# smithlabcode/abismal

Measured on AMD Instinct MI355X. Metric: mapped reads/sec (whole node), 100 bp SE on hg38-scale index, higher is better.
Workload: dtype u64

## Files before the change

### abismal_amd/csrc/abm_kernels.hip

```cpp
#include <type_traits>
#include "abm_kernels_core.hpp"
#include "abm_sam.hpp"

#ifndef ABM_SE_WAVES_PER_SIMD
#define ABM_SE_WAVES_PER_SIMD 5
#endif


namespace abm {

__global__ __launch_bounds__(256) void pack_reads_kernel(const char *__restrict__ blob,
                                                         const u64 *__restrict__ off, u64 n_reads,
                                                         u32 W, u64 *__restrict__ packed,
                                                         u32 *__restrict__ lens) {
  const u64 gid = static_cast<u64>(blockIdx.x) * blockDim.x + threadIdx.x;
  const u64 r = gid / W;
  const u32 w = static_cast<u32>(gid % W);
  if (r >= n_reads)
    return;
  const u64 b = off[r];
  const u32 L = static_cast<u32>(off[r + 1] - b);
  if (w == 0)
    lens[r] = L;
  u64 ft = 0, fa = 0, rt = 0, ra = 0;
// ... 30 lines not shown
  if (b >= n_blocks) return;
  u64 lo = 0, hi = 0;
  bool multi = false, blank = false;
  for (u32 k = 0; k < 4; ++k) {
    const u64 w = 4 * b + k;
    const u64 x = w < n_words ? genome[w] : 0ull;
    lo |= static_cast<u64>(every_fourth_bit((x >> 1) | (x >> 3))) << (16 * k);
    hi |= static_cast<u64>(every_fourth_bit((x >> 2) | (x >> 3))) << (16 * k);
    const u64 ones = (x & 0x1111111111111111ull) + ((x >> 1) & 0x1111111111111111ull) +
                     ((x >> 2) & 0x1111111111111111ull) + ((x >> 3) & 0x1111111111111111ull);
    u64 part = 0x1111111111111111ull;
    const u64 first = 16 * w;
    if (first >= n_bases) part = 0;
    else if (n_bases - first < 16) part &= (1ull << (4 * (n_bases - first))) - 1;
    if (ones & (part * 14ull)) multi = true;
    if ((~(ones | (ones >> 1) | (ones >> 2)) & part) != 0) blank = true;
  }
  p0[2 * b] = lo; p0[2 * b + 1] = hi;
  p1[2 * b] = lo; p1[2 * b + 1] = hi;
  if (multi) atomicOr(bad, 1u);
  if (blank) {
    const u64 at = b * kPlaneBlock, from = at >= kPlaneReach ? at - kPlaneReach : 0;
    for (u64 c = from >> kPlaneChunkBits; c <= (at + kPlaneBlock - 1) >> kPlaneChunkBits; ++c)
      atomicOr(&nmap[c >> 5], 1u << (c & 31u));
  }
}

template <bool BAM>
__device__ __forceinline__ u32 format_sam_tail(const SeArgs &a, u8 *line , const u32 *fin, u64 r,
                                               u32 L, const Hit &best, u32 n_ops) {
  const bool ambig = (best.flags & kFlagAmbig) != 0;
  if (best.pos == 0 || L == 0 || (ambig && !a.sam_allow_ambig)) return 0;
  if (n_ops == 0 || n_ops > a.cig_stride || n_ops > kSeCap) return 0xFFFFFFFFu;
  wave_sync();
  const u32 reflen = sam_ref_len(fin, n_ops);
  u32 chrom = 0, c0 = 0;
  if (!sam_locate(a.ix, best.pos, reflen, chrom, c0)) return 0;
  const bool rc = (best.flags & kFlagRC) != 0;
  const u32 flag = (rc ? 0x10u : 0u) | ((a.sam_allow_ambig && ambig) ? 0x100u : 0u);
  if constexpr (BAM) {
    const BamFields f{static_cast<int>(chrom) - 1, best.pos - c0, reflen, flag, -1, 0u, 0, best.diffs, (best.flags & kFlagARich) != 0};
    return BamWriter{line, a.sam_stride}.write(f, fin, n_ops, a.blob + a.off[r], L, rc, a.sam_tail + r * a.sam_stride);
  }
  SamWriter o{line, 0, a.sam_stride};
  o.put('\t');
  o.put_uint(flag);
  o.put('\t');
  o.put_chrom(a.ix, chrom);
  o.put('\t');
  o.put_uint(best.pos - c0 + 1u);
  o.put_str("\t255\t", 5);
  o.put_cigar(fin, n_ops);
  o.put_str("\t*\t0\t0\t", 7);
  o.put_seq(a.blob + a.off[r], L, rc);
  o.put_tags(best.diffs, (best.flags & kFlagARich) != 0);
  if (o.w > o.cap) return 0xFFFFFFFFu;
  o.flush(reinterpret_cast<u32 *>(a.sam_tail + r * a.sam_stride));
  return o.w;
}

template <bool TIMED, bool COOP, bool LONG, bool REC = false, bool BAM = false>
__device__ __forceinline__ void map_se_body(const SeArgs &a) {
  extern __shared__ __align__(16) unsigned char smem[];
  const int lane = lane_id();
  WaveLds lds;
  lds.W = a.W;
  lds.WB = a.WB;
  lds.qpk = reinterpret_cast<u64 *>(smem);
  lds.GW = a.GW;
  lds.qbits = lds.qpk + 4 * a.W;
  lds.MB = LONG ? 0u : (a.max_len + kPlaneBlock - 1) / kPlaneBlock;
  lds.qmask = lds.qbits + 4 * a.WB;
  lds.max_jobs = LONG ? 2u : kMaxJobs;
  {
    unsigned char *p = reinterpret_cast<unsigned char *>(lds.qmask + 4 * lds.MB * 4);
    const u32 cap2 = (a.ctmp_cap + 1) & ~1u;
    if (LONG) lds.ctmp = a.long_ctmp + static_cast<u64>(blockIdx.x) * cap2;
    else { lds.ctmp = reinterpret_cast<u32 *>(p); p += cap2 * 4; }
    lds.jpos = reinterpret_cast<u32 *>(p); p += kSeCap * 4;
    lds.jdf = reinterpret_cast<u32 *>(p); p += kSeCap * 4;
    lds.gwin = reinterpret_cast<u64 *>(p); p += lds.max_jobs * a.GW * 8;
    lds.pcache = reinterpret_cast<u64 *>(p); p += (8u << kPosCacheBits) + (LONG ? 0u : a.tb_extra);
    lds.tb = LONG ? a.long_tb + static_cast<u64>(blockIdx.x) * a.long_tb_bytes : reinterpret_cast<u8 *>(lds.gwin + a.GW);
    lds.lbest = reinterpret_cast<int *>(p); p += 64 * 4;
    lds.smark = reinterpret_cast<u32 *>(p); p += 128 * 4;
    lds.sdelta = reinterpret_cast<u32 *>(p); p += 128 * 4;
    lds.mark = reinterpret_cast<u16 *>(p);
  }
  lds.hres = reinterpret_cast<u16 *>(lds.lbest);
  lds.G = a.G;
  lds.smark[lane] = 0; lds.smark[64 + lane] = 0;
  u32 seg_epoch = 0;

  const u32 n_calls = a.mode == 2 ? 4u : 2u;
  const u32 call_rc = a.mode == 2 ? 0xCu  : 0x2u ;
  const u32 call_ar = a.mode == 2 ? 0x6u  : (a.mode == 1 ? 0x3u : 0x0u);

  WorkTally wt = {0, 0, 0, 0, 0, 0, 0, 0, 0, 0, 0, 0, 0, 0};
  const CigarSink sink = {a.cig_stride, a.ctmp_cap, a.cig_arena, a.cig_arena_count, a.cig_arena_cap, (!LONG && a.sam_tail) ? lds.jpos : nullptr};
  const u64 n_items = a.n_reads;
  long long t_begin = 0, t_a = 0, t_b = 0;
  ABM_STAMP(t_begin);
  u32 n_aln = 0, n_single = 0;
  bool overflow = false, too_long = false;

  const u64 dealt = gridDim.x;
  auto next_read = [&]() -> u64 {
    unsigned long long v = 0;
    if (lane == 0) {
      v = atomicAdd(a.next_read, 1ull) + dealt;
      if (v >= n_items && a.drained) __hip_atomic_store(a.drained, 1u, __ATOMIC_RELAXED, __HIP_MEMORY_SCOPE_SYSTEM);
    }
    return (static_cast<u64>(static_cast<u32>(uni(static_cast<int>(v >> 32)))) << 32) |
           static_cast<u32>(uni(static_cast<int>(v)));
  };
  u64 r_next = blockIdx.x;
  while (r_next < n_items) {
    const u64 slot = r_next;
    const u64 r = a.order ? static_cast<u64>(a.order[r_next]) : r_next;
    r_next = next_read();
    __builtin_amdgcn_s_setprio(0);
    long long t_read = 0;
    if (TIMED) t_read = clock64();
    bool rd_overflow = false;
    const u32 L = a.lens[r];
    Hit best;
    best.diffs = 0x7fff; best.flags = 0; best.pos = 0;
    u32 n_ops = 0;
    u32 *cig_out = a.cig + r * a.cig_stride;
    if (L > kMaxReadLen) too_long = true;
    if (L >= a.ix.min_len && L <= a.max_len) {
      const u64 *src = a.packed + (LONG ? slot : r) * 4 * a.W;
      for (u32 k = lane; k < 4 * a.W; k += 64) lds.qpk[k] = src[k];
      wave_sync();
      for (u32 e = 0; e < 4; ++e)
        for (u32 wb = 0; wb < a.WB; ++wb) {
          const u32 j = wb * 64 + lane;
          const bool b = j < L ? bit2(q_nibble(lds.qpk + e * a.W, j)) : true;
          const u64 word = __ballot(b);
          if (lane == 0) lds.qbits[e * a.WB + wb] = word;
        }
      if constexpr (COOP) build_qmasks(lds, L);
      wave_sync();
      if (L < max(a.ix.window, L >> 1) + kKeyWeight - 1)
        ghost_bits(a.packed, a.lens, r, L, a.max_len, a.ix.min_len, a.W, a.WB, lds.qbits);

      SeSet S;
      S.begin_read(L);
      for (u32 cidx = 0; cidx < n_calls; ++cidx) {
        const bool rc = (call_rc >> cidx) & 1u, ar = (call_ar >> cidx) & 1u;
        const bool g_to_a = rc != ar;
        const u32 enc = (rc ? 2u : 0u) + (g_to_a ? 1u : 0u);
        const u32 flags = (rc ? kFlagRC : 0u) | (ar ? kFlagARich : 0u);
        S.cutoff = S.good_cutoff;
        seed_pass<true, TIMED, COOP, REC>(a.ix, lds, enc, g_to_a, flags, L, S, wt, seg_epoch);
        if (S.sz != static_cast<int>(kSeCap) || S.cutoff > S.good_cutoff) {
          S.cutoff = S.top_d();
          seed_pass<false, TIMED, COOP, REC>(a.ix, lds, enc, g_to_a, flags, L, S, wt, seg_epoch);
        }
      }
      ABM_STAMP(t_a);
      choose_se<LONG>(a.ix, lds, L, a.valid_frac, S, best, cig_out, sink, n_ops, rd_overflow, n_aln, n_single);
      overflow |= rd_overflow;
      ABM_STAMP(t_b);
      if (TIMED) wt.t_align += t_b - t_a;
    }
    if constexpr (!LONG) {
      if (a.sam_tail != nullptr) {
        const u32 len = (L > a.max_len) ? 0xFFFFFFFFu : format_sam_tail<BAM>(a, lds.tb, lds.jpos, r, (L >= a.ix.min_len) ? L : 0u, best, best.pos != 0 ? n_ops : 0u);
        if (lane == 0) store_out(a.sam_len + r, len);
      }
    }
    if (lane == 0) {
      store_out(a.res + r, best);
      store_out(a.cig_n + r, best.pos != 0 ? n_ops : 0u);
      if (TIMED && a.read_cycles) a.read_cycles[r] = static_cast<u32>((clock64() - t_read) >> 10);
    }
    if (!LONG && a.slice_left != nullptr) {
      __builtin_amdgcn_fence(__ATOMIC_RELEASE, "workgroup");
      asm volatile("s_waitcnt vmcnt(0)" ::: "memory");
      if (lane == 0 && !rd_overflow) {
        const u32 sl = a.slice_id[r];
        if (sl != 0xFFFFu && atomicSub(&a.slice_left[sl], 1u) == 1u) {
          __threadfence_system();
          __hip_atomic_store(a.slice_done + sl, 1u, __ATOMIC_RELAXED, __HIP_MEMORY_SCOPE_SYSTEM);
        }
      }
    }
  }
  if (TIMED && a.work) {
    auto wsum = [&](u32 v) { u32 t; (void)wave_excl_sum(v, t); return t; };
    const u32 s0 = wsum(wt.seed_iters), s1 = wsum(wt.probes), s2 = wsum(wt.cands), s3 = wsum(wt.words);
    const u32 wsum_hits = wsum(wt.cache_hits);
    if (lane == 0) {
      atomicAdd(&a.work[0], static_cast<unsigned long long>(s0));
      atomicAdd(&a.work[1], static_cast<unsigned long long>(s1));
      atomicAdd(&a.work[2], static_cast<unsigned long long>(s2));
      atomicAdd(&a.work[3], static_cast<unsigned long long>(s3));
      atomicAdd(&a.work[4], static_cast<unsigned long long>(wt.updates));
      atomicAdd(&a.work[5], static_cast<unsigned long long>(n_aln));
      atomicAdd(&a.work[11], static_cast<unsigned long long>(wsum_hits));
      atomicAdd(&a.work[12], static_cast<unsigned long long>(n_single));
      if (TIMED) {
        atomicAdd(&a.work[6], static_cast<unsigned long long>(wt.t_probe));
        atomicAdd(&a.work[7], static_cast<unsigned long long>(wt.t_stream));
        atomicAdd(&a.work[8], static_cast<unsigned long long>(wt.t_replay));
        atomicAdd(&a.work[9], static_cast<unsigned long long>(wt.t_align));
        atomicAdd(&a.work[10], static_cast<unsigned long long>(phase_stamp() - t_begin));
        atomicAdd(&a.work[13], static_cast<unsigned long long>(wt.light_steps));
        atomicAdd(&a.work[14], static_cast<unsigned long long>(wt.fifo_updates));
        atomicAdd(&a.work[15], static_cast<unsigned long long>(wt.steps));
      }
    }
  }
  if (lane == 0 && (overflow || too_long))
    atomicOr(a.status, (overflow ? 1u : 0u) | (too_long ? 2u : 0u));
  if (a.host_tail != nullptr && lane == 0) {
    __threadfence();
    const u32 before = atomicAdd(a.finished, 1u);
    if (before + 1u == gridDim.x) {
      __threadfence();
      a.host_tail[0] = __hip_atomic_load(a.cig_arena_count, __ATOMIC_RELAXED, __HIP_MEMORY_SCOPE_AGENT);
      a.host_tail[1] = __hip_atomic_load(a.status, __ATOMIC_RELAXED, __HIP_MEMORY_SCOPE_AGENT);
    }
  }
}

template <bool TIMED, bool COOP, bool REC = false>
__global__ __launch_bounds__(64, ABM_SE_WAVES_PER_SIMD) void map_se_kernel(SeArgs a) { map_se_body<TIMED, COOP, false, REC>(a); }
template <bool COOP, bool REC>
__global__ __launch_bounds__(64, ABM_SE_WAVES_PER_SIMD) void map_se_bam_kernel(SeArgs a) { map_se_body<false, COOP, false, REC, true>(a); }
__global__ __launch_bounds__(64, 1) void map_se_long_kernel(SeArgs a) { map_se_body<false, false, true>(a); }

__global__ __launch_bounds__(256) void collect_long_kernel(const u32 *__restrict__ lens, u64 n, u32 *__restrict__ list,
                                                           u32 *__restrict__ count) {
  const u64 r = static_cast<u64>(blockIdx.x) * blockDim.x + threadIdx.x;
  if (r < n && lens[r] > kLdsReadLen && lens[r] <= kMaxReadLen) list[atomicAdd(count, 1u)] = static_cast<u32>(r);
}
__global__ __launch_bounds__(256) void pack_listed_kernel(const char *__restrict__ blob, const u64 *__restrict__ off,
                                                          const u32 *__restrict__ list, u64 m, u32 W, u64 *__restrict__ packed) {
  const u64 gid = static_cast<u64>(blockIdx.x) * blockDim.x + threadIdx.x;
  const u64 slot = gid / W;
  const u32 w = static_cast<u32>(gid % W);
  if (slot >= m) return;
  const u64 r = list[slot];
  const u64 b = off[r];
  const u32 L = static_cast<u32>(off[r + 1] - b);
  u64 ft = 0, fa = 0, rt = 0, ra = 0;
  for (u32 j = 0; j < 16; ++j) {
    const u32 k = w * 16 + j;
    u32 nft = 15, nfa = 15, nrt = 15, nra = 15;
    if (k < L) {
      const u32 cf = static_cast<u8>(blob[b + k]);
      const u32 cr = comp_base(static_cast<u8>(blob[b + (L - 1 - k)]));
      nft = read_nibble(cf, false); nfa = read_nibble(cf, true);
      nrt = read_nibble(cr, false); nra = read_nibble(cr, true);
    }
    const u32 sh = j << 2;
    ft |= static_cast<u64>(nft) << sh; fa |= static_cast<u64>(nfa) << sh;
    rt |= static_cast<u64>(nrt) << sh; ra |= static_cast<u64>(nra) << sh;
  }
  if (w * 16 >= L) ft = fa = rt = ra = ~0ull;
  u64 *dst = packed + (slot * 4) * W + w;
  dst[0] = ft; dst[W] = fa; dst[2 * W] = rt; dst[3 * W] = ra;
}

__device__ __forceinline__ u32 weight_class(const DevIndex &ix, const u64 *pk, u32 L, bool g_to_a) {
  u32 k2 = 0, k3 = 0;
  const u64 w0 = pk[0], w1 = L > 16 ? pk[1] : 0ull;
  for (u32 j = 0; j < kKeyWeight; ++j) {
    const u32 nb = static_cast<u32>((j < 16 ? w0 >> (j << 2) : w1 >> ((j - 16) << 2))) & 15u;
    k2 = (k2 << 1) | bit2(nb);
  }
  for (u32 j = 0; j < kKeyWeight3; ++j)
    k3 = k3 * 3u + trit(static_cast<u32>(w0 >> (j << 2)) & 15u, g_to_a);
  const u32 *cnt3 = g_to_a ? ix.counter_a : ix.counter_t;
  const u32 occ = (ix.counter[k2 + 1] - ix.counter[k2]) + (cnt3[k3 + 1] - cnt3[k3]);
  return 32u - static_cast<u32>(__clz(static_cast<int>(occ | 1u)));
}

__global__ __launch_bounds__(256) void weigh_reads_kernel(DevIndex ix, const u64 *__restrict__ packed,
                                                          const u32 *__restrict__ lens, u64 n, u32 W,
                                                          int mode, u8 *__restrict__ cls,
                                                          u32 *__restrict__ class_count) {
  __shared__ u32 hist[33];
  if (threadIdx.x < 33) hist[threadIdx.x] = 0;
  __syncthreads();
  const u64 r = static_cast<u64>(blockIdx.x) * blockDim.x + threadIdx.x;
  if (r < n) {
    const u32 L = lens[r];
    u32 c = 0;
    if (L >= ix.min_len) {
      const u64 *pk = packed + r * 4 * W;
      const bool ar = mode == 1;
      c = max(weight_class(ix, pk + (ar ? 1 : 0) * W, L, ar), weight_class(ix, pk + (2 + (ar ? 0 : 1)) * W, L, !ar));
    }
    cls[r] = static_cast<u8>(c);
    atomicAdd(&hist[c], 1u);
  }
  __syncthreads();
  if (threadIdx.x < 33 && hist[threadIdx.x]) atomicAdd(&class_count[threadIdx.x], hist[threadIdx.x]);
}

__global__ void order_bases_kernel(u32 *class_count ) {
  if (threadIdx.x == 0 && blockIdx.x == 0) {
    u32 at = 0;
    for (int c = 32; c >= 0; --c) { const u32 k = class_count[c]; class_count[c] = at; at += k; }
// ... 283 lines not shown
```

### abismal_amd/csrc/abm_kernels_core.hpp

```cpp
#pragma once
#include "abm_kernels.hpp"

namespace abm {

struct SeSet {
  static constexpr bool kFifo = true;
  static constexpr bool kAppend = false;
  int hk;
  u32 pf;
  u32 pp;
  int sz, cutoff, good_cutoff;
  int best_d;
  u32 best_f, best_p;
  bool sure_ambig;

  __device__ __forceinline__ static int key_d(int k) { return k >> 8; }
  __device__ __forceinline__ void begin_read(u32 readlen) {
    const int worst = static_cast<i16>(0.4 * readlen);
    hk = worst * 256; pf = 0; pp = 0;
    sz = 1;
    cutoff = worst;
    good_cutoff = static_cast<i16>(readlen / 10u);
    best_d = worst; best_f = 0; best_p = 0;
    sure_ambig = false;
  }
  __device__ __forceinline__ int top_d() const { return key_d(rdlane(hk, 0)); }
  __device__ __forceinline__ void sift_up(int hole, int key) {
    int parent = (hole - 1) / 2;
    while (hole > 0) {
      const int pk = rdlane(hk, parent);
      if (!(key_d(pk) < key_d(key))) break;
      wrlane(hk, hole, pk);
      hole = parent;
      parent = (hole - 1) / 2;
    }
    wrlane(hk, hole, key);
  }
  __device__ __forceinline__ int pop_max(int n) {
    const int len = n - 1;
    const int freed = rdlane(hk, 0) & 255;
    const int vk = rdlane(hk, len);
    int hole = 0, second = 0;
    while (second < (len - 1) / 2) {
      second = 2 * (second + 1);
      int sk = rdlane(hk, second);
      const int lk = rdlane(hk, second - 1);
      if (key_d(sk) < key_d(lk)) { --second; sk = lk; }
      wrlane(hk, hole, sk);
      hole = second;
    }
    if ((len & 1) == 0 && second == (len - 2) / 2) {
      second = 2 * (second + 1);
      wrlane(hk, hole, rdlane(hk, second - 1));
      hole = second - 1;
    }
    sift_up(hole, vk);
    return freed;
  }
  __device__ __forceinline__ int replace_top(int d, u32 f, u32 p) {
    static_assert(kSeCap == 50, "paths derived for a 50-element heap");
    const int left = __builtin_amdgcn_update_dpp(0, hk, 0x138 , 0xf, 0xf, false);
    const u64 right_wins = __ballot(!(key_d(hk) < key_d(left)));
    auto down = [&](int node) { const int r = 2 * node + 2; return ((right_wins >> r) & 1ull) ? r : r - 1; };
    const int root = rdlane(hk, 0), vk = rdlane(hk, 49);
    const int p1 = down(0), p2 = down(p1), p3 = down(p2), p4 = down(p3);
    const bool five = p4 < 24;
    const int p5 = five ? down(p4) : 63;
    const int k1 = rdlane(hk, p1), k2 = rdlane(hk, p2), k3 = rdlane(hk, p3), k4 = rdlane(hk, p4), k5 = rdlane(hk, p5);
    const int dv = key_d(vk);
    int j = 0;
    if (key_d(k1) >= dv) j = 1;
    if (key_d(k2) >= dv) j = 2;
    if (key_d(k3) >= dv) j = 3;
    if (key_d(k4) >= dv) j = 4;
    if (five && key_d(k5) >= dv) j = 5;
    wrlane(hk, 0, j == 0 ? vk : k1);
    wrlane(hk, p1, j > 1 ? k2 : (j == 1 ? vk : k1));
    wrlane(hk, p2, j > 2 ? k3 : (j == 2 ? vk : k2));
    wrlane(hk, p3, j > 3 ? k4 : (j == 3 ? vk : k3));
    wrlane(hk, p4, j > 4 ? k5 : (j == 4 ? vk : k4));
    wrlane(hk, p5, j == 5 ? vk : k5);
    const int slot = root & 255;
    wrlane(pf, slot, f);
    wrlane(pp, slot, p);
    const int nk = d * 256 + slot;
    const int c24 = rdlane(hk, 24), c11 = rdlane(hk, 11), c5 = rdlane(hk, 5), c2 = rdlane(hk, 2), c0 = rdlane(hk, 0);
    const bool b24 = key_d(c24) < d, b11 = b24 && key_d(c11) < d, b5 = b11 && key_d(c5) < d, b2 = b5 && key_d(c2) < d,
               b0 = b2 && key_d(c0) < d;
    wrlane(hk, 49, b24 ? c24 : nk);
    wrlane(hk, 24, b24 ? (b11 ? c11 : nk) : c24);
    wrlane(hk, 11, b11 ? (b5 ? c5 : nk) : c11);
    wrlane(hk, 5, b5 ? (b2 ? c2 : nk) : c5);
    wrlane(hk, 2, b2 ? (b0 ? c0 : nk) : c2);
    const int top = b0 ? nk : c0;
    wrlane(hk, 0, top);
    return top;
  }

  __device__ __forceinline__ int tie_run(u64 &todo, u64 ties, u32 cand_pos, u32 f) {
    static_assert(kSeCap == 50, "paths derived for a 50-element heap");
    const int lane = lane_id();
    const int c = cutoff;
    if (sz != static_cast<int>(kSeCap) || key_d(rdlane(hk, 0)) != c || key_d(rdlane(hk, 24)) != c || key_d(rdlane(hk, 49)) != c)
      return 0;
    const u64 brk = todo & ~ties;
    u64 run = brk ? (todo & ((brk & (0 - brk)) - 1)) : todo;
    if (run == 0) return 0;
    const int m = __popcll(run);
    todo &= ~run;
    const int left = __builtin_amdgcn_update_dpp(0, hk, 0x138 , 0xf, 0xf, false);
    const u64 right_wins = __ballot(!(key_d(hk) < key_d(left)));
    auto down = [&](int node) { const int r = 2 * node + 2; return ((right_wins >> r) & 1ull) ? r : r - 1; };
    const int p1 = down(0), p2 = down(p1), p3 = down(p2), p4 = down(p3);
    const int p5 = p4 < 24 ? down(p4) : 63;
    const bool e1 = key_d(rdlane(hk, p1)) == c, e2 = e1 && key_d(rdlane(hk, p2)) == c, e3 = e2 && key_d(rdlane(hk, p3)) == c,
               e4 = e3 && key_d(rdlane(hk, p4)) == c, e5 = e4 && p4 < 24 && key_d(rdlane(hk, p5)) == c;
    const int n = 2 + (e1 ? 1 : 0) + (e2 ? 1 : 0) + (e3 ? 1 : 0) + (e4 ? 1 : 0) + (e5 ? 1 : 0);
    int src = lane;
    wrlane(src, 0, e1 ? p1 : 49);
    if (e1) wrlane(src, p1, e2 ? p2 : 49);
    if (e2) wrlane(src, p2, e3 ? p3 : 49);
    if (e3) wrlane(src, p3, e4 ? p4 : 49);
    if (e4) wrlane(src, p4, e5 ? p5 : 49);
    if (e5) wrlane(src, p5, 49);
    int play = m;
    while (play >= 2 * n) play -= n;
    u64 last = 0, rest = run;
    for (int k = 0; k < play; ++k) {
      const int top = 63 - __builtin_clzll(rest);
      last |= 1ull << top;
      rest &= ~(1ull << top);
    }
    const int c256 = c * 256;
    while (last) {
      const int l = __builtin_ctzll(last);
      last &= last - 1;
      const int slot = rdlane(hk, 0) & 255;
      const u32 p = rdlane(cand_pos, l);
      hk = __builtin_amdgcn_ds_bpermute(src << 2, hk);
      wrlane(hk, 49, c256 + slot);
      wrlane(pp, slot, p);
      wrlane(pf, slot, f);
    }
    return m;
  }

  __device__ __forceinline__ void admit(bool specific, int d, u32 f, u32 p) {
    if (d == 0) {
      if (best_p == 0) { best_d = 0; best_f = f; best_p = p; }
      else if (p != best_p || f != best_f) best_f |= kFlagAmbig;
    }
    int top;
    if (d != 0 && sz == static_cast<int>(kSeCap)) top = key_d(replace_top(d, f, p));
    else {
      if (d != 0) {
        const int slot = sz++;
        wrlane(pf, slot, f);
        wrlane(pp, slot, p);
        sift_up(sz - 1, d * 256 + slot);
      }
      top = top_d();
    }
    sure_ambig = (best_f & kFlagAmbig) && best_d == 0;
    cutoff = specific ? min(cutoff, top) : top;
  }
};

struct WaveLds {
  u64 *qpk;
  u64 *qbits;
  u64 *qmask;
  u16 *mark;
  u32 *smark;
  u32 *sdelta;
  u32 *ctmp;
  u8 *tb;
  u64 *gwin;
  u32 *jpos;
  u32 *jdf;
  int *lbest;
  u64 *pcache;
  u16 *hres;
  u32 W, WB, GW, MB;
  u32 G;
  u32 max_jobs;
};
constexpr u32 kPosCacheBits = 8;
constexpr u32 kMaxJobs = 21;

__device__ __forceinline__ u32 q_nibble(const u64 *qpk, u32 k) {
  return static_cast<u32>(qpk[k >> 4] >> ((k & 15u) << 2)) & 15u;
}

__device__ __forceinline__ u64 q_window16(const u64 *qpk, u32 W, u32 i, u32 L) {
  const u32 w = i >> 4, s = (i & 15u) << 2;
  u64 x = qpk[w] >> s;
  if (s && w + 1 < W) x |= qpk[w + 1] << (64 - s);
  const u32 have = i < L ? min(16u, L - i) : 0u;
  if (have < 16) x &= (have == 0 ? 0ull : ((1ull << (have << 2)) - 1));
  return x;
}

__device__ __forceinline__ u32 genome_bit2(const DevIndex &ix, u64 q) { return bit2(gnib(ix.genome, q)); }
__device__ __forceinline__ u32 genome_sortsym3(const DevIndex &ix, u64 q, bool g_to_a) { return sortsym3(gnib(ix.genome, q), g_to_a); }

__device__ __forceinline__ u32 record_nibble(const DevIndex &ix, const u32 *__restrict__ tbl, u32 rec0, bool live, u32 k, u32 p) {
  const u32 at = ix.wrec_back + p, last = ix.wrec_blocks * 64u - 1u;
  const bool in_reach = at < last;
  const u64 *r = ix.wrec + 2ull * (live ? static_cast<u64>(k + rec0) * ix.wrec_blocks : 0ull);
  const u32 blk = in_reach ? at >> 6 : 0u;
  const u64 lo = r[2 * blk], hi = r[2 * blk + 1], flag = r[2 * (ix.wrec_blocks - 1)];
  u32 nib = 1u << ((static_cast<u32>(lo >> (at & 63u)) & 1u) | ((static_cast<u32>(hi >> (at & 63u)) & 1u) << 1));
  if (live && (!in_reach || (flag >> 63))) nib = gnib(ix.genome, static_cast<u64>(tbl[k]) + p);
  return nib;
}
template <bool REC = false>
__device__ __forceinline__ void narrow_both(const DevIndex &ix, const u32 *__restrict__ tbl3, bool g_to_a, const u64 *qb,
                                            u32 n_bits, const u64 *qpk, u32 qbase, u32 limit, u32 maxc, bool run2, u32 &lo2,
                                            u32 &hi2, u32 &len2, bool run3, u32 &lo3, u32 &hi3, u32 &len3, u32 &probes, u32 rec3 = 0) {
  const u32 *__restrict__ tbl2 = ix.index;
  const u32 mid_sym = g_to_a ? 2u : 1u, top_sym = g_to_a ? 8u : 4u;
  u32 pA = len2, ploA = lo2, phiA = hi2, blA = 0;
  int bnA = 0;
  auto goA = [&]() { return pA != limit && (hi2 - lo2) > maxc && qbase + pA < n_bits + 4096u; };
  bool actA = run2 && goA();
  if (actA) { blA = lo2; bnA = static_cast<int>(hi2 - lo2); }
  u32 pB = len3, ploB = lo3, phiB = hi3, l1 = 0, l2 = 0;
  int n1 = 0, n2 = 0;
  auto goB = [&]() { return pB != limit && (hi3 - lo3) > maxc; };
  bool actB = run3 && goB();
  if (actB) { l1 = l2 = lo3; n1 = n2 = static_cast<int>(hi3 - lo3); }
  while (actA || actB) {
    const int hA = bnA >> 1, h1 = n1 >> 1, h2 = n2 >> 1;
    const u32 kA = blA + static_cast<u32>(hA), m1 = l1 + static_cast<u32>(h1), m2 = l2 + static_cast<u32>(h2);
    const bool dA = actA, d1 = actB && n1 > 0, d2 = actB && n2 > 0 && !(d1 && m2 == m1);
    u32 sA, s1, s2;
    if constexpr (REC) {
      sA = bit2(record_nibble(ix, tbl2, 0u, dA, kA, pA));
      s1 = sortsym3(record_nibble(ix, tbl3, rec3, d1, m1, pB), g_to_a);
      s2 = sortsym3(record_nibble(ix, tbl3, rec3, d2, m2, pB), g_to_a);
    }
    else {
      const u32 eA = tbl2[dA ? kA : 0u], e1 = tbl3[d1 ? m1 : 0u], e2 = tbl3[d2 ? m2 : 0u];
      sA = genome_bit2(ix, static_cast<u64>(eA) + pA);
      s1 = genome_sortsym3(ix, static_cast<u64>(e1) + pB, g_to_a);
      s2 = genome_sortsym3(ix, static_cast<u64>(e2) + pB, g_to_a);
    }
    probes += (dA ? 1u : 0u) + (d1 ? 1u : 0u) + (d2 ? 1u : 0u);
    if (actA) {
      if (sA < 1u) { blA = kA + 1; bnA -= hA + 1; } else bnA = hA;
      if (bnA <= 0) {
        const u32 at = qbase + pA;
        const bool one = at < n_bits ? ((qb[at >> 6] >> (at & 63u)) & 1ull) != 0 : true;
        lo2 = one ? blA : lo2;
        hi2 = one ? hi2 : blA;
        ++pA;
        actA = goA();
        if (actA) { ploA = lo2; phiA = hi2; blA = lo2; bnA = static_cast<int>(hi2 - lo2); }
      }
    }
    if (actB) {
      if (n2 > 0 && n1 > 0 && m2 == m1) s2 = s1;
      if (n1 > 0) { if (s1 < mid_sym) { l1 = m1 + 1; n1 -= h1 + 1; } else n1 = h1; }
      if (n2 > 0) { if (s2 < top_sym) { l2 = m2 + 1; n2 -= h2 + 1; } else n2 = h2; }
      if (n1 <= 0 && n2 <= 0) {
        const u32 sym = sortsym3(q_nibble(qpk, qbase + pB), g_to_a);
        const u32 nlo = sym == 0 ? lo3 : (sym == mid_sym ? l1 : l2), nhi = sym == 0 ? l1 : (sym == mid_sym ? l2 : hi3);
        lo3 = nlo;
        hi3 = nhi;
        ++pB;
        actB = goB();
        if (actB) { ploB = lo3; phiB = hi3; l1 = l2 = lo3; n1 = n2 = static_cast<int>(hi3 - lo3); }
      }
    }
  }
  if (run2 && lo2 == hi2) { --pA; lo2 = ploA; hi2 = phiA; }
  if (run3 && lo3 == hi3) { --pB; lo3 = ploB; hi3 = phiB; }
  len2 = pA;
  len3 = pB;
}

__device__ __forceinline__ u32 every_fourth_bit(u64 t) {
  t &= 0x1111111111111111ull;
  t = (t | (t >> 3)) & 0x0303030303030303ull;
  t = (t | (t >> 6)) & 0x000F000F000F000Full;
  t = (t | (t >> 12)) & 0x000000FF000000FFull;
  t = (t | (t >> 24)) & 0xFFFFull;
  return static_cast<u32>(t);
}

__device__ __forceinline__ void classes16(int mode, u64 x, u32 &c1, u32 &c2) {
  const u64 y = mode == 1 ? x : x >> 1;
  c2 = every_fourth_bit(y >> 2);
  c1 = every_fourth_bit(y & ~(y >> 2));
}
__device__ __forceinline__ void read_classes64(int mode, const u64 *qb, u32 n_bits, const u64 *qpk, u32 W, u32 L, u32 s, u64 &r1, u64 &r2) {
  if (mode == 0) {
    const u32 w = s >> 6, sh = s & 63u;
    const u64 a = s < n_bits ? qb[w] : ~0ull, b = s + 64 < n_bits ? qb[w + 1] : ~0ull;
    r1 = sh ? (a >> sh) | (b << (64 - sh)) : a;
    r2 = 0;
    return;
  }
  r1 = r2 = 0;
#pragma unroll
  for (u32 j = 0; j < 4; ++j) {
    u32 c1, c2;
    classes16(mode, q_window16(qpk, W, s + 16 * j, L), c1, c2);
    r1 |= static_cast<u64>(c1) << (16 * j);
    r2 |= static_cast<u64>(c2) << (16 * j);
  }
}
struct DirectArgs { const u64 *planes0; const u32 *nmap; const u64 *qb; const u64 *qpk; u32 n_bits, W, L, maxc; };
struct DirectRange { u32 lo, hi, len, probes; bool ok; };
__device__ __forceinline__ DirectRange narrow_direct(int mode, DirectArgs da, const u32 *__restrict__ tbl, u32 qbase, u32 limit, u32 lo, u32 hi, u32 len) {
  const u64 *qb = da.qb, *qpk = da.qpk;
  const u32 n_bits = da.n_bits, W = da.W, L = da.L, maxc = da.maxc;
// ... 362 lines not shown
      qbits[e * WB + 1] = (m >> (64 - L)) | (~0ull << L);
    }
  }
  wave_sync();
}

#ifndef ABM_SE_DIRECT_NARROWING
#define ABM_SE_DIRECT_NARROWING true
#endif
#ifndef ABM_SE_RECORD_PROBES
#define ABM_SE_RECORD_PROBES false
#endif
#ifndef ABM_HEAVY_BLOCK
#define ABM_HEAVY_BLOCK 4096
#endif
constexpr u32 kHeavyBlock = ABM_HEAVY_BLOCK;
struct WorkTally {
  u32 seed_iters, probes, cands, words, updates, cache_hits;
  u32 fifo_updates, steps, light_steps;
  long long t_probe, t_stream, t_replay, t_align, t_total;
};
__device__ __forceinline__ long long phase_stamp() {
  unsigned long long t;
  __builtin_amdgcn_sched_barrier(0);
  asm volatile("s_waitcnt vmcnt(0) lgkmcnt(0)\n\ts_memtime %0\n\ts_waitcnt lgkmcnt(0)" : "=s"(t) : : "memory");
  __builtin_amdgcn_sched_barrier(0);
  return static_cast<long long>(t);
}
#define ABM_STAMP(var) do { if (TIMED) var = phase_stamp(); } while (0)

template <bool SPECIFIC, bool TIMED, bool COOP, bool REC, class Set>
__device__ __forceinline__ void seed_pass(const DevIndex &ix, const WaveLds &lds, u32 enc, bool g_to_a,
                                          u32 flags, u32 L, Set &S, WorkTally &wt, u32 &seg_epoch) {
  const int lane = lane_id();
  const u64 *qpk = lds.qpk + enc * lds.W;
  const u64 *qb = lds.qbits + enc * lds.WB;
  const u32 *cnt3 = g_to_a ? ix.counter_a : ix.counter_t;
  const u32 *idx3 = g_to_a ? ix.index_a : ix.index_t;
  const u32 maxc = ix.max_candidates;
  const u32 nwords = (L + 15) >> 4;
  const u32 spec_len = min(L - ix.window, L >> 1);
  const u32 n_off = SPECIFIC ? max(ix.window, L >> 1) : L - kKeyWeight + 1;
  const bool use_ext = SPECIFIC && ix.ext2 != nullptr && ix.ext_maxc == maxc &&
                       L - n_off + 1 >= max(kKeyWeight + ix.e2, kKeyWeight3 + ix.e3);
  static_assert(!REC || COOP, "window records are filtered cooperatively");
  const u32 rec3 = g_to_a ? ix.wrec_a0 : ix.wrec_t0;

  constexpr bool TALLY = TIMED;
  constexpr bool kDirect = Set::kAppend ? ABM_PE_DIRECT_NARROWING : ABM_SE_DIRECT_NARROWING;
  long long ta = 0, tb_ = 0, tc = 0, td = 0;
  if (SPECIFIC && !REC) {
    for (u32 k = lane; k < (1u << kPosCacheBits); k += 64) lds.pcache[k] = 0;
    wave_sync();
  }
  for (u32 g0 = 0; g0 < n_off && !S.sure_ambig; g0 += 64) {
      ABM_STAMP(ta);
    const u32 i = g0 + lane;
    const bool live = i < n_off;
    u32 lo2 = 0, hi2 = 0, lo3 = 0, hi3 = 0;
    bool chk2 = false, chk3 = false;
    if (live) {
      const u32 wq = i >> 6, sq = i & 63u;
      u64 bits = qb[wq] >> sq;
      if (sq) bits |= qb[wq + 1] << (64 - sq);
      const u32 k2 = __brev(static_cast<u32>(bits) & 0x1FFFFFFu) >> 7;
      const u64 win = q_window16(qpk, lds.W, i, L);
      u32 k3 = 0;
#pragma unroll
      for (u32 j = 0; j < 16; ++j)
        k3 = k3 * 3u + trit(static_cast<u32>(win >> (j << 2)) & 15u, g_to_a);
      if (SPECIFIC) {
        u32 probes = 0;
        u32 len2 = kKeyWeight, len3 = kKeyWeight3;
        bool run2 = true, run3 = true;
        if (use_ext) {
          const u32 D2 = kKeyWeight + ix.e2;
          const u32 K2 = __brev(static_cast<u32>(bits) & (D2 >= 32 ? 0xFFFFFFFFu : (1u << D2) - 1u)) >> (32 - D2);
          const u64 more = q_window16(qpk, lds.W, i + 16, L);
          u32 K3 = k3;
          for (u32 j = 0; j < ix.e3; ++j) K3 = K3 * 3u + trit(static_cast<u32>(more >> (j << 2)) & 15u, g_to_a);
          const uint2 x2 = ix.ext2[K2], x3 = (g_to_a ? ix.ext3a : ix.ext3t)[K3];
          const u32 st2 = x2.y >> 30, st3 = x3.y >> 30;
          lo2 = x2.x; hi2 = x2.x + (x2.y & 0x7FFFFFFu); len2 = kKeyWeight + ((x2.y >> 27) & 7u); run2 = st2 != 0;
          lo3 = x3.x; hi3 = x3.x + (x3.y & 0x7FFFFFFu); len3 = kKeyWeight3 + ((x3.y >> 27) & 7u); run3 = st3 != 0;
          if (st2 == 2) { lo2 = ix.counter[k2]; hi2 = ix.counter[k2 + 1]; len2 = kKeyWeight; }
          if (st3 == 2) { lo3 = cnt3[k3]; hi3 = cnt3[k3 + 1]; len3 = kKeyWeight3; }
        }
        else {
          lo2 = ix.counter[k2]; hi2 = ix.counter[k2 + 1];
          lo3 = cnt3[k3];       hi3 = cnt3[k3 + 1];
        }
        if constexpr (kDirect) {
          if (ix.direct_min != 0 && L <= kSortDepth && ix.planes[0] != nullptr) {
            const u32 limit = L - i;
            const DirectArgs da = {ix.planes[0], ix.nmap, qb, qpk, 64u * lds.WB, lds.W, L, maxc};
#pragma unroll 1
            for (int chain = 0; chain < 2; ++chain) {
              const bool three = chain != 0;
              const u32 clo = three ? lo3 : lo2, chi = three ? hi3 : hi2, clen = three ? len3 : len2;
              if ((three ? run3 : run2) && chi - clo >= ix.direct_min && chi - clo > maxc && clen < limit) {
                const DirectRange r = narrow_direct(three ? (g_to_a ? 2 : 1) : 0, da, three ? idx3 : ix.index, i, limit, clo, chi, clen);
                probes += r.probes;
                if (r.ok) {
                  if (three) { lo3 = r.lo; hi3 = r.hi; len3 = r.len; run3 = false; }
                  else { lo2 = r.lo; hi2 = r.hi; len2 = r.len; run2 = false; }
                }
              }
            }
          }
        }
        narrow_both<REC && (Set::kAppend || ABM_SE_RECORD_PROBES)>(ix, idx3, g_to_a, qb, 64u * lds.WB, qpk, i, L - i, maxc, run2, lo2, hi2, len2, run3, lo3, hi3, len3, probes, rec3);
        chk2 = (hi2 - lo2) <= maxc || len2 >= spec_len;
        chk3 = (hi3 - lo3) <= maxc || len3 >= spec_len;
        if (TALLY) wt.probes += probes;
      }
      else {
        lo2 = ix.counter[k2]; hi2 = ix.counter[k2 + 1];
        lo3 = cnt3[k3];       hi3 = cnt3[k3 + 1];
        const u32 d2 = hi2 - lo2, d3 = hi3 - lo3;
        chk2 = d2 != 0 && d2 <= maxc && (d3 == 0 || d2 <= 10u * d3);
        chk3 = d3 != 0 && d3 <= maxc;
      }
      if (TALLY) ++wt.seed_iters;
    }
    Segs sg;
    sg.na = chk2 ? hi2 - lo2 : 0u;
    sg.nb = chk3 ? hi3 - lo3 : 0u;
    sg.lo2 = lo2;
    sg.lo3 = lo3;
    if constexpr (TALLY && Set::kAppend) {
      if (sg.na) wt.words += ((lo2 + sg.na - 1) >> 5) - (lo2 >> 5) + 1;
      if (sg.nb) wt.words += ((lo3 + sg.nb - 1) >> 5) - (lo3 >> 5) + 1;
    }
    u32 total;
    sg.start_a = wave_excl_sum(sg.na + sg.nb, total);
    ABM_STAMP(tb_);
    if (TIMED) wt.t_probe += tb_ - ta;
    if (total == 0) continue;
    if (total >= kHeavyBlock) __builtin_amdgcn_s_setprio(3);
    if (seg_epoch >= kSegEpochLimit) {
      lds.smark[lane] = 0; lds.smark[64 + lane] = 0;
      seg_epoch = 0;
    }
    publish_segs(lds, sg);

    auto replay = [&](bool valid, int h, int hmax, u32 pos) {
      u64 todo = __ballot(valid && hmax <= S.cutoff);
      if constexpr (Set::kAppend) if (SPECIFIC && !S.heaped && todo) {
        const int offered = __popcll(todo);
        todo = S.append(todo, h, pos);
        if (TALLY) wt.updates += static_cast<u32>(offered - __popcll(todo));
      }
      while (todo && !S.sure_ambig) {
        if constexpr (Set::kFifo) {
          const int applied = S.tie_run(todo, __ballot(valid && h == S.cutoff), pos, flags);
          if (applied) {
            if (TALLY) wt.updates += static_cast<u32>(applied);
            if (TIMED) wt.fifo_updates += static_cast<u32>(applied);
            continue;
          }
        }
        const int l = __builtin_ctzll(todo);
        const int before = S.cutoff;
        S.admit(true, rdlane(h, l), flags, rdlane(pos, l));
        if (TALLY) ++wt.updates;
        todo &= ~(((1ull << l) << 1) - 1);
        if (S.cutoff < before) todo &= __ballot(valid && hmax <= S.cutoff);
      }
    };

    if constexpr (REC) {
      u32 carry = 0;
      for (u32 c0 = 0; c0 < total && !S.sure_ambig; c0 += 128) {
        ABM_STAMP(tc);
        if (TIMED) { ++wt.steps; if (total - c0 <= 64) ++wt.light_steps; }
        const bool two = c0 + 64 < total;
        bool va, vb;
        u32 sa, sb, ea, eb;
        locate128(lds, seg_epoch, sg, c0, total, carry, va, vb, sa, sb, ea, eb);
        const u32 ia = g0 + (sa >> 1), ib = g0 + (sb >> 1);
        const u32 ra = (ea + ((sa & 1u) ? rec3 : 0u)) * ix.wrec_blocks, rb = (eb + ((sb & 1u) ? rec3 : 0u)) * ix.wrec_blocks;
        int ha, hb = 0x7fff;
        if (lds.G == 2)
          hamming_records_lane<false>(ix, lds.qmask + enc * lds.MB * 4, L, ra, ix.wrec_back - ia, va, rb, ix.wrec_back - ib, vb, two, ha, hb);
        else
          hamming_records_lane<true>(ix, lds.qmask + enc * lds.MB * 4, L, ra, ix.wrec_back - ia, va, rb, ix.wrec_back - ib, vb, two, ha, hb);
        const bool ca = va && ha <= S.cutoff, cb = two && vb && hb <= S.cutoff;
        u32 pa = 0, pb = 0;
        if (__any(ca || cb)) {
          if (ca) pa = ((sa & 1u) ? idx3[ea] : ix.index[ea]) - ia;
          if (cb) pb = ((sb & 1u) ? idx3[eb] : ix.index[eb]) - ib;
          const u32 na = ca ? ix.nmap[pa >> (kPlaneChunkBits + 5)] >> ((pa >> kPlaneChunkBits) & 31u) : 0u;
          const u32 nb = cb ? ix.nmap[pb >> (kPlaneChunkBits + 5)] >> ((pb >> kPlaneChunkBits) & 31u) : 0u;
          if (__any((na | nb) & 1u)) {
            if (na & 1u) ha = hamming(ix.genome, qpk, nwords, pa);
            if (nb & 1u) hb = hamming(ix.genome, qpk, nwords, pb);
          }
        }
        if (TALLY) {
          wt.cands += (va ? 1u : 0u) + (vb ? 1u : 0u);
          if constexpr (!Set::kAppend) wt.words += ((va ? 1u : 0u) + (vb ? 1u : 0u)) * (lds.G == 2 ? 6u : 8u);
        }
        ABM_STAMP(td);
        if (TIMED) wt.t_stream += td - tc;
        replay(ca, ha, ha, pa);
        if (two && !S.sure_ambig) replay(cb, hb, hb, pb);
        ABM_STAMP(tc);
        if (TIMED) wt.t_replay += tc - td;
      }
      continue;
    }
    u32 carry = 0;
    bool nva = false, nvb = false;
    u32 nsa = 0, nsb = 0, nea = 0, neb = 0;
    auto fetch_entries = [&](u32 c0) {
      u32 ea_at, eb_at;
      locate128(lds, seg_epoch, sg, c0, total, carry, nva, nvb, nsa, nsb, ea_at, eb_at);
      nea = 0; neb = 0;
      if (nva) nea = (nsa & 1u) ? idx3[ea_at] : ix.index[ea_at];
      if (nvb) neb = (nsb & 1u) ? idx3[eb_at] : ix.index[eb_at];
    };
    fetch_entries(0);
    for (u32 c0 = 0; c0 < total && !S.sure_ambig; c0 += 128) {
          ABM_STAMP(tc);
      if (TIMED) { ++wt.steps; if (total - c0 <= 64) ++wt.light_steps; }
      const bool two = c0 + 64 < total;
      const bool va = nva, vb = nvb;
      const u32 pa = nea - (g0 + (nsa >> 1)), pb = neb - (g0 + (nsb >> 1));
      if (c0 + 128 < total) fetch_entries(c0 + 128);
      u64 *slot_a = lds.pcache + ((pa * 2654435761u) >> (32 - kPosCacheBits));
      u64 *slot_b = lds.pcache + ((pb * 2654435761u) >> (32 - kPosCacheBits));
      const u64 ca = va ? *slot_a : 0ull, cb = vb ? *slot_b : 0ull;
      const bool hit_a = va && static_cast<u32>(ca) == pa, hit_b = vb && static_cast<u32>(cb) == pb;
      int ha, hma, hb = 0x7fff, hmb = 0x7fff;
      if constexpr (COOP) {
        const u32 na = va && !hit_a ? ix.nmap[pa >> (kPlaneChunkBits + 5)] >> ((pa >> kPlaneChunkBits) & 31u) : 0u;
        const u32 nb = vb && !hit_b ? ix.nmap[pb >> (kPlaneChunkBits + 5)] >> ((pb >> kPlaneChunkBits) & 31u) : 0u;
        if (lds.G == 2)
          hamming_planes_pairs(ix, lds, lds.qmask + enc * lds.MB * 4, L, pa, va && !hit_a, pb, vb && !hit_b, ha, hb);
        else
          hamming_planes(ix, lds, lds.qmask + enc * lds.MB * 4, L, pa, va && !hit_a, pb, vb && !hit_b, ha, hb);
        if (__any((na | nb) & 1u)) {
          if (na & 1u) ha = hamming(ix.genome, qpk, nwords, pa);
          if (nb & 1u) hb = hamming(ix.genome, qpk, nwords, pb);
        }
        hma = ha; hmb = hb;
      }
      else
        hamming2(ix.genome, qpk, nwords, pa, va && !hit_a, pb, vb && !hit_b, ha, hma, hb, hmb);
      if (hit_a) { ha = static_cast<i16>(static_cast<u16>(ca >> 32)); hma = static_cast<i16>(static_cast<u16>(ca >> 48)); }
      if (va && !hit_a)
        *slot_a = static_cast<u64>(pa) | (static_cast<u64>(static_cast<u16>(ha)) << 32) | (static_cast<u64>(static_cast<u16>(hma)) << 48);
      if (!va) { ha = hma = 0x7fff; }
      if (two) {
        if (hit_b) { hb = static_cast<i16>(static_cast<u16>(cb >> 32)); hmb = static_cast<i16>(static_cast<u16>(cb >> 48)); }
        if (vb && !hit_b)
          *slot_b = static_cast<u64>(pb) | (static_cast<u64>(static_cast<u16>(hb)) << 32) | (static_cast<u64>(static_cast<u16>(hmb)) << 48);
        if (!vb) { hb = hmb = 0x7fff; }
      }
      if (TALLY) {
      wt.cands += (va ? 1u : 0u) + (vb ? 1u : 0u);
      const u32 fetched = COOP ? (lds.G == 2 ? 6u : (lds.G == 4 ? 8u : 2u * ((L + kPlaneBlock - 1) / kPlaneBlock + 1))) : nwords;
      if constexpr (!Set::kAppend) wt.words += ((va ? 1u : 0u) + (vb ? 1u : 0u)) * fetched;
      wt.cache_hits += (hit_a ? 1u : 0u) + (hit_b ? 1u : 0u);
      }
      ABM_STAMP(td);
      if (TIMED) wt.t_stream += td - tc;
      replay(va, ha, hma, pa);
      if (two && !S.sure_ambig) replay(vb, hb, hmb, pb);
      ABM_STAMP(tc);
      if (TIMED) wt.t_replay += tc - td;
    }
  }
}

__device__ __forceinline__ int band_for(int diffs, int max_diffs) {
  const int v = 2 * min(diffs, max_diffs) + 1;
  return v < 0 ? static_cast<int>(kMaxBand) : min(static_cast<int>(kMaxBand), v);
}
__device__ __forceinline__ int from_prev_lane(int v) {
  return __builtin_amdgcn_update_dpp(0, v, 0x138 , 0xf, 0xf, true);
}
__device__ __forceinline__ int from_next_lane(int v) {
  return __builtin_amdgcn_update_dpp(0, v, 0x130 , 0xf, 0xf, true);
}

__device__ __forceinline__ u64 nibbles16(const u64 *words, int nwords, int start) {
  if (start <= -16 || start >= 16 * nwords)
    return 0ull;
  if (start < 0)
    return words[0] << ((-start) << 2);
  const int w = start >> 4, s = (start & 15) << 2;
  u64 x = words[w] >> s;
  if (s && w + 1 < nwords) x |= words[w + 1] << (64 - s);
  return x;
}

struct AlnJob {
  int bw;
  int jl;
  int qoff;
  int g;
  int t0nib;
};

template <bool WRAP> __device__ __forceinline__ int score16(int v) { return WRAP ? static_cast<int>(static_cast<i16>(v)) : v; }
// ... 629 lines not shown
```

Measured before the change: 22.57 million.

## Short-circuit SE candidate set updates once an exact hit is found

Once an exact (distance 0) hit exists, the single-end candidate set stops maintaining its heap of inexact hits. It only counts them until capacity is reached, then drops the cutoff to zero so later seeds can only test for ambiguity. A wave-wide after_exact path settles a whole batch of candidates with ballots instead of admitting them one by one. When the set is already full with a best hit, set_specific starts later passes at cutoff 0. The aim is to cut per-candidate admit and heap work after an exact match. The risk is that heap contents and the non-zero candidates used later (e.g., in choose_se) are no longer maintained, which could change mapping output.

```diff
diff --git a/abismal_amd/csrc/abm_kernels.hip b/abismal_amd/csrc/abm_kernels.hip
--- a/abismal_amd/csrc/abm_kernels.hip
+++ b/abismal_amd/csrc/abm_kernels.hip
@@ -206,7 +206,7 @@
         const bool g_to_a = rc != ar;
         const u32 enc = (rc ? 2u : 0u) + (g_to_a ? 1u : 0u);
         const u32 flags = (rc ? kFlagRC : 0u) | (ar ? kFlagARich : 0u);
-        S.cutoff = S.good_cutoff;
+        S.set_specific();
         seed_pass<true, TIMED, COOP, REC>(a.ix, lds, enc, g_to_a, flags, L, S, wt, seg_epoch);
         if (S.sz != static_cast<int>(kSeCap) || S.cutoff > S.good_cutoff) {
           S.cutoff = S.top_d();
diff --git a/abismal_amd/csrc/abm_kernels_core.hpp b/abismal_amd/csrc/abm_kernels_core.hpp
--- a/abismal_amd/csrc/abm_kernels_core.hpp
+++ b/abismal_amd/csrc/abm_kernels_core.hpp
@@ -145,10 +145,32 @@
     return m;
   }
 
+  __device__ __forceinline__ bool settled() const { return best_p != 0 && sz == static_cast<int>(kSeCap); }
+  __device__ __forceinline__ void set_specific() { cutoff = settled() ? 0 : good_cutoff; }
+  __device__ __forceinline__ int after_exact(u64 todo, int h, u32 cand_pos, u32 f) {
+    const bool mine = (todo >> lane_id()) & 1ull;
+    const u64 zeros = __ballot(mine && h == 0);
+    const u64 other = __ballot(mine && h == 0 && (cand_pos != best_p || f != best_f));
+    if (other) {
+      best_f |= kFlagAmbig;
+      sure_ambig = true;
+      todo &= ((other & (0 - other)) << 1) - 1;
+    }
+    const int grow = min(static_cast<int>(kSeCap) - sz, __popcll(todo & ~zeros));
+    sz += grow;
+    if (sz == static_cast<int>(kSeCap)) cutoff = 0;
+    return __popcll(todo & zeros) + grow;
+  }
+
   __device__ __forceinline__ void admit(bool specific, int d, u32 f, u32 p) {
     if (d == 0) {
       if (best_p == 0) { best_d = 0; best_f = f; best_p = p; }
       else if (p != best_p || f != best_f) best_f |= kFlagAmbig;
+    }
+    else if (best_p != 0) {
+      sz = min(sz + 1, static_cast<int>(kSeCap));
+      if (sz == static_cast<int>(kSeCap)) cutoff = 0;
+      return;
     }
     int top;
     if (d != 0 && sz == static_cast<int>(kSeCap)) top = key_d(replace_top(d, f, p));
@@ -163,6 +185,7 @@
     }
     sure_ambig = (best_f & kFlagAmbig) && best_d == 0;
     cutoff = specific ? min(cutoff, top) : top;
+    if (d == 0 && sz == static_cast<int>(kSeCap)) cutoff = 0;
   }
 };
 
@@ -831,6 +854,13 @@
         if (TALLY) wt.updates += static_cast<u32>(offered - __popcll(todo));
       }
       while (todo && !S.sure_ambig) {
+        if constexpr (!Set::kAppend) {
+          if (S.best_p != 0) {
+            const int played = S.after_exact(todo, h, pos, flags);
+            if (TALLY) wt.updates += static_cast<u32>(played);
+            break;
+          }
+        }
         if constexpr (Set::kFifo) {
           const int applied = S.tie_run(todo, __ballot(valid && h == S.cutoff), pos, flags);
           if (applied) {
```

Result: no change. 22.53 million, median of 2 (-0.2%).
